# zhangyi-3/UCDIR

Measured on AMD Instinct MI355X. Metric: restored images/sec at 50-step p_sample_loop, 256x256 SID, higher is better.
Workload: dtype bf16

## Files before the change

### ucdir_amd/csrc/akgm_ws64.hip.h

```cpp
#pragma once
#include "asmops.hip.h"
#include "akgm_ws32.hip.h"

struct AkWs64 {
    static constexpr int NW = 8;
    static constexpr int HPOS = 272;
    static constexpr int HALO = HPOS * 128;
    static constexpr int HBYTES(int hpos) { return ((hpos + 15) / 16) * 2048; }
    static constexpr int PSTEP = 32 * 128;
    static constexpr int SEGB = 8 * NW;
    static constexpr int CPS = SEGB / 16;
    static constexpr int STAGE = 128 * SEGB;
    static constexpr int ATT = 128 * 32;
    static constexpr int TCS = 9 * 32 * NW * 4;
    static constexpr int NK = 36;
    static constexpr int lds(int hpos) { return 2 * HBYTES(hpos) + 2 * STAGE + 2 * ATT + TCS; }
};

template <int NPT, int NW, bool ASYM>
__global__ __launch_bounds__(64 * NW, 2) void akgm_ws64_kernel(const AkgmHP p) {
    static_assert(NW == AkWs64::NW && ASYM, "akgm_ws64_kernel: only the eight-wave kind with the chores on waves 0 - 3 is built");
    using L = AkWs64;
    constexpr int NK = L::NK;
    constexpr int CPX = 512;
    constexpr int NPX = 32 * NPT;
    constexpr int FEAT = 4 * NW;
    constexpr int PP = 1024 / L::SEGB;
    constexpr int NDW = 4;
    extern __shared__ __attribute__((aligned(16))) unsigned char smem[];
    const int tid = threadIdx.x, lane = tid & 63, l31 = lane & 31, hh = lane >> 5;
    const int wave = __builtin_amdgcn_readfirstlane(tid >> 6);
    int lid;
    {
        const int nblk = gridDim.x, bid = blockIdx.x;
        const int q = nblk >> 3, r = nblk & 7, xcd = bid & 7;
        lid = (xcd < r ? xcd * (q + 1) : r * (q + 1) + (xcd - r) * q) + (bid >> 3);
    }
#ifndef W64_DBGWAVE
#define W64_DBGWAVE (NW - 3)
#endif
#ifdef UCDIR_TIMING
    const bool dbg_on = p.dbg && (lid == (int)gridDim.x / 2 + 3) && (lane == 0) && (wave == W64_DBGWAVE);
    int dbg_n = 0;
#define W64_STAMP() do { if (dbg_on && dbg_n < 250) p.dbg[dbg_n++] = __builtin_amdgcn_s_memtime(); } while (0)
#else
#define W64_STAMP() do {} while (0)
#endif
    W64_STAMP();
    constexpr int NROLE = 512 / FEAT;
    const int nslots = (int)gridDim.x / NROLE;
    const int role = lid / nslots, slot = lid - role * nslots;
    const int Wp = p.Wp, Ptot = (p.H + 2) * Wp, Plast = p.H * Wp + p.W;
    const float inv_wp = 1.0f / (float)Wp;
    const int tps = p.tiles_x, T = p.nbatch * tps;
    const int t_beg = (int)((long long)slot * T / nslots), t_end = (int)((long long)(slot + 1) * T / nslots);
    if (t_beg >= t_end) return;
    const int chan0 = FEAT * role;
    const int gch0 = 64 * (chan0 >> 6);
    const int HB = p.tw;
    const unsigned OFF_STAGE = 2 * HB, OFF_ATT = OFF_STAGE + 2 * L::STAGE, OFF_TCS = OFF_ATT + 2 * L::ATT;

    bf16x8_t af[NK];
    {
        const unsigned char* Ab = reinterpret_cast<const unsigned char*>(p.A) + ((long long)(role * NW + wave) * NK) * 1024 + lane * 16;
#pragma unroll
        for (int j = 0; j < NK; ++j) af[j] = *reinterpret_cast<const bf16x8_t*>(Ab + j * 1024);
    }
#pragma unroll
    for (int j = 0; j < NK; ++j) asm volatile("" : "+v"(af[j]));
    W64_STAMP();

    const int npiece = (NPX + 2 * Wp + 2 + 7) >> 3;
    constexpr int NHOP = (L::HPOS / 8 + NDW - 1) / NDW;
    constexpr int NROP = NW / NDW;
    unsigned bt[9];
#pragma unroll
    for (int t = 0; t < 9; ++t) {
        const int hp = l31 + (t / 3) * Wp + t % 3;
        bt[t] = hp * 128 + ((hh ^ ((hp >> 1) & 7)) << 4) + HB;
    }
    const unsigned tc_lane = OFF_TCS + 4 * 8 * (4 * wave + 2 * hh);
    const unsigned att_lane = OFF_ATT + l31 * 32;
    const unsigned st_lane = OFF_STAGE + l31 * L::SEGB + (((wave >> 1) ^ ((l31 >> 2) & (L::CPS - 1))) << 4) + 8 * (wave & 1) + 4 * hh;

    int b = t_beg / tps, ti = t_beg - b * tps;
    auto dma_op = [&](auto opc, int nb, int nti, int buf) {
        constexpr int op = decltype(opc)::value;
        unsigned ln = lane;
        asm volatile("" : "+v"(ln));
        if constexpr (op < NHOP) {
            const int k = op * NDW + wave;
            if (k < npiece) {
                int sp = nti * NPX + 8 * k + (int)(ln >> 3);
                sp = sp < Ptot ? sp : Ptot - 1;
                const unsigned off = (unsigned)sp * (CPX * 2) + (unsigned)(gch0 + (((ln & 7) ^ (4 * (k & 1) + (ln >> 4))) << 3)) * 2;
                dma16_sbase(p.h + (long long)nb * p.h_bstride, off, (unsigned)__builtin_amdgcn_readfirstlane(buf * HB + k * 1024));
            }
        } else if constexpr (op == NHOP) {
            if (wave < NPT) {
                int P = Wp + 1 + nti * NPX + 32 * wave + (int)(ln >> 1); P = P < Ptot ? P : Ptot - 1;
                int y = fdiv_small(P, inv_wp), x = P - y * Wp;
                y = y < 1 ? 1 : (y > p.H ? p.H : y); x = x < 1 ? 1 : (x > p.W ? p.W : x);
                dma16_sbase(p.G + (long long)nb * p.g_bstride, (unsigned)((((y - 1) * p.W + (x - 1)) * 8 + (int)(ln & 1) * 4) * 4),
                          (unsigned)__builtin_amdgcn_readfirstlane(OFF_ATT + buf * L::ATT + wave * 1024));
            }
        } else {
            constexpr int rk = op - NHOP - 1;
            const int piece = NDW * rk + wave;
            if (piece < NPX / PP) {
                const unsigned pos = PP * piece + ln / L::CPS;
                int P = Wp + 1 + nti * NPX + (int)pos; P = P < Ptot ? P : Ptot - 1;
                const unsigned off = (unsigned)P * (CPX * 2) + (unsigned)(chan0 + (((ln & (L::CPS - 1)) ^ ((pos >> 2) & (L::CPS - 1))) << 3)) * 2;
                dma16_sbase(p.res + (long long)nb * p.res_bstride, off, (unsigned)__builtin_amdgcn_readfirstlane(OFF_STAGE + buf * L::STAGE + piece * 1024));
            }
        }
    };
    constexpr int NOPS = NHOP + 1 + NROP;
    if (wave < NDW) static_for<0, NOPS>([&](auto opc) { dma_op(opc, b, ti, 0); });

    int b_cur = -1;
    float rstd = 1.f, aw[8];
#pragma unroll
    for (int s = 0; s < 8; ++s) aw[s] = 0.f;
    stat_t S1 = 0, S2 = 0;
    bool have_prev = false;
    long long prev_out[NROP];
#pragma unroll
    for (int i = 0; i < NROP; ++i) prev_out[i] = -1;

#pragma unroll 1
    for (int t = t_beg; t <= t_end; ++t) {
        const int buf = (t - t_beg) & 1;
        W64_STAMP();
        asm volatile("s_waitcnt vmcnt(0) lgkmcnt(0)\n\ts_barrier" ::: "memory");
        W64_STAMP();
        if (have_prev && wave < NDW) {
#pragma unroll
            for (int i = 0; i < NROP; ++i) {
                if (prev_out[i] >= 0) {
                    const u32x4_t ln = *reinterpret_cast<const u32x4_t*>(smem + OFF_STAGE + (buf ^ 1) * L::STAGE + (i * 64 * NDW + tid) * 16);
                    *reinterpret_cast<u32x4_t*>(reinterpret_cast<unsigned char*>(p.out) + prev_out[i]) = ln;
                }
            }
        }
        if (t == t_end) break;
        if (b != b_cur) {
            if (b_cur >= 0 && p.stats_out) {
                const stat_t a = wave_sum_ll(S1), q2 = wave_sum_ll(S2);
                if (lane == 0) stat_add_fx(p.stats_out, b_cur, a, q2);
            }
            S1 = 0; S2 = 0;
            b_cur = b;
            float mean_b = 0.f;
            if (p.own_tc) stat_mean_rstd_wave(p.stats, b, p.inv_count, lane, mean_b, rstd);
            else rstd = __builtin_bit_cast(float, __builtin_amdgcn_readfirstlane(__builtin_bit_cast(int, p.ms[2 * b + 1])));
            const float inv_b = 1.0f / rstd;
#pragma unroll
            for (int i = 0; i < (9 + NW - 1) / NW; ++i) {
                const int pc = i * NW + wave;
                if (pc < 9) {
                    const long long rel = (long long)pc * (8 * CPX) + 8 * chan0 + lane * 4;
                    if (p.own_tc) akgm_tc_piece(p, rel, smem + OFF_TCS + pc * 1024 + lane * 16, inv_b, mean_b);
                    else __builtin_amdgcn_global_load_lds((const GLOBAL_AS void*)(p.Tc + (long long)b * 9 * (8 * CPX) + rel),
                                                          (LDS_AS void*)(smem + OFF_TCS + pc * 1024), 16, 0, 0);
                }
            }
#pragma unroll
            for (int s = 0; s < 8; ++s) aw[s] = __builtin_bit_cast(float, __builtin_amdgcn_readfirstlane(__builtin_bit_cast(int, p.attw[b * 8 + s])));
            asm volatile("s_waitcnt vmcnt(0) lgkmcnt(0)\n\ts_barrier" ::: "memory");
        }
        const bool last = t + 1 == t_end;
        int nb = b, nti = ti + 1;
        if (nti == tps) { nti = 0; ++nb; }
        asm volatile("s_waitcnt lgkmcnt(0)" ::: "memory");
        W64_STAMP();
        if (!last && wave < NDW) static_for<0, NOPS>([&](auto opc) { dma_op(opc, nb, nti, buf ^ 1); });

        const int P0 = Wp + 1 + ti * NPX;
        const unsigned ab0 = buf * L::ATT, sb0 = buf * L::STAGE;
#pragma unroll
        for (int k = 0; k < 9; ++k) bt[k] = buf ? bt[k] + HB : bt[k] - HB;
        float s1 = 0.f, s2 = 0.f;
#pragma unroll 1
        for (int qp = 0; qp < NPT; qp += 2) {
            f32x16_t acc[2];
            bool valid[2];
#pragma unroll
            for (int tq = 0; tq < 2; ++tq) {
                const int P = P0 + 32 * (qp + tq) + l31;
                const int y = fdiv_small(P, inv_wp), x = P - y * Wp;
                valid[tq] = x >= 1 && x <= p.W && P <= Plast;
                const int cy = (y <= 1) ? 0 : ((y >= p.H) ? 2 : 1);
                const int cx = (x <= 1) ? 0 : ((x >= p.W) ? 2 : 1);
                const unsigned tca = tc_lane + (cy * 3 + cx) * (128 * NW);
                acc[tq] = lds_read_f32x16(smem + tca);
            }
            bf16x8_t bfr[3][2];
            __builtin_amdgcn_sched_barrier(0);
            asm volatile("s_waitcnt lgkmcnt(0)" ::: "memory");
            W64_STAMP();
            auto frag = [&](auto jc, bf16x8_t (&dst)[2]) {
                constexpr int j = decltype(jc)::value;
                const unsigned a0 = bt[j >> 2] ^ ((j & 3) << 5);
                lds_read16_asm<0>(dst[0], a0);
                lds_read16_asm<L::PSTEP>(dst[1], a0);
            };
            frag(std::integral_constant<int, 0>{}, bfr[0]);
            frag(std::integral_constant<int, 1>{}, bfr[1]);
            __builtin_amdgcn_s_setprio(1);
            static_for<0, NK>([&](auto jc) {
                constexpr int j = decltype(jc)::value;
                if constexpr (j + 2 < NK) frag(std::integral_constant<int, j + 2>{}, bfr[(j + 2) % 3]);
                constexpr int younger = (j + 2 < NK) ? 4 : ((j + 1 < NK) ? 2 : 0);
                lgkm_wait_asm<younger>();
#pragma unroll
                for (int tq = 0; tq < 2; ++tq) acc[tq] = __builtin_amdgcn_mfma_f32_32x32x16_bf16(af[j], bfr[j % 3][tq], acc[tq], 0, 0, 0);
            });
            __builtin_amdgcn_s_setprio(0);
            W64_STAMP();
#pragma unroll
            for (int tq = 0; tq < 2; ++tq) {
                const unsigned aq = att_lane + ab0 + (qp + tq) * 1024;
                const f32x4_t a0 = *reinterpret_cast<const f32x4_t*>(smem + aq), a1 = *reinterpret_cast<const f32x4_t*>(smem + aq + 16);
                const float att[8] = {a0[0] * aw[0], a0[1] * aw[1], a0[2] * aw[2], a0[3] * aw[3], a1[0] * aw[4], a1[1] * aw[5], a1[2] * aw[6], a1[3] * aw[7]};
                float o2[2];
#pragma unroll
                for (int k = 0; k < 2; ++k) {
                    float sa = 0.f;
#pragma unroll
                    for (int s = 0; s < 8; ++s) sa += att[s] * acc[tq][8 * k + s];
                    o2[k] = rstd * sa;
                }
                const unsigned sa = st_lane + sb0 + (qp + tq) * (32 * L::SEGB);
                const unsigned rv = *reinterpret_cast<const unsigned*>(smem + sa);
                float v0 = silu_fast(o2[0]) + __builtin_bit_cast(float, rv << 16);
                float v1 = silu_fast(o2[1]) + __builtin_bit_cast(float, rv & 0xffff0000u);
                *reinterpret_cast<unsigned*>(smem + sa) = pack2_bf16(v0, v1);
                v0 = valid[tq] ? v0 : 0.f; v1 = valid[tq] ? v1 : 0.f;
                s1 += v0 + v1; s2 += v0 * v0 + v1 * v1;
            }
#pragma unroll
            for (int k = 0; k < 9; ++k) bt[k] += 2 * L::PSTEP;
        }
#pragma unroll
        for (int k = 0; k < 9; ++k) bt[k] -= NPT * L::PSTEP;
        S1 += stat_fx((double)s1); S2 += stat_fx((double)s2);
        have_prev = true;
        if (wave < NDW) {
#pragma unroll
            for (int i = 0; i < NROP; ++i) {
                const int it = i * 64 * NDW + tid, mpos = it / L::CPS, P = P0 + mpos;
                const int y = fdiv_small(P < Ptot ? P : Ptot - 1, inv_wp), x = P - y * Wp;
                const bool ok = mpos < NPX && x >= 1 && x <= p.W && P <= Plast;
                prev_out[i] = ok ? ((long long)b * p.out_bstride + (long long)P * CPX + chan0 + (((it & (L::CPS - 1)) ^ ((mpos >> 2) & (L::CPS - 1))) << 3)) * 2 : -1;
            }
        }
        b = nb; ti = nti;
    }
#ifdef UCDIR_TIMING
    if (dbg_on) p.dbg[255] = dbg_n;
#endif
    if (p.stats_out) {
        const stat_t a = wave_sum_ll(S1), q2 = wave_sum_ll(S2);
        if (lane == 0) stat_add_fx(p.stats_out, b_cur, a, q2);
    }
}
```

### ucdir_amd/csrc/pack.h

```cpp
#pragma once
#include <cmath>
#include <cstdint>
#include <vector>

#include "common.h"

struct PackedConv {
    std::vector<bf16_t> A;
    std::vector<float> bias;
    std::vector<float> Tb, Tg;
    int rows_pad = 0, Kpad = 0, ntaps = 0, cin = 0, cout = 0, ncls = 0;
};

static inline bool tap_valid(int cls, int tap) {
    const int cy = cls / 3, cx = cls % 3, ky = tap / 3, kx = tap % 3;
    if (cy == 0 && ky == 0) return false;
    if (cy == 2 && ky == 2) return false;
    if (cx == 0 && kx == 0) return false;
    if (cx == 2 && kx == 2) return false;
    return true;
}

static inline PackedConv pack_conv(const float* w, const float* bias, const float* gamma, const float* beta,
                                   int cout, int cin, int ks, int TM) {
    PackedConv P;
    P.ntaps = ks * ks; P.cin = cin; P.cout = cout;
    P.Kpad = ((P.ntaps * cin + 63) / 64) * 64;
    P.rows_pad = ((cout + TM - 1) / TM) * TM;
    P.A.assign((size_t)P.rows_pad * P.Kpad, 0);
    P.bias.assign(P.rows_pad, 0.f);
    if (bias) for (int o = 0; o < cout; ++o) P.bias[o] = bias[o];
    P.ncls = (ks == 3) ? 9 : 1;
    const bool fold = gamma != nullptr;
    std::vector<double> wb((size_t)P.ntaps * cout, 0.0), wg((size_t)P.ntaps * cout, 0.0);
    for (int o = 0; o < cout; ++o)
        for (int c = 0; c < cin; ++c)
            for (int t = 0; t < P.ntaps; ++t) {
                const float wv = w[((size_t)o * cin + c) * P.ntaps + t];
                const float ws = fold ? wv * gamma[c] : wv;
                const bf16_t q = f2bf(ws);
                P.A[(size_t)o * P.Kpad + (size_t)t * cin + c] = q;
                if (fold) {
                    wb[(size_t)t * cout + o] += (double)wv * beta[c];
                    wg[(size_t)t * cout + o] += (double)bf2f(q);
                }
            }
    if (fold) {
        P.Tb.assign((size_t)P.ncls * cout, 0.f);
        P.Tg.assign((size_t)P.ncls * cout, 0.f);
        for (int cls = 0; cls < P.ncls; ++cls)
            for (int o = 0; o < cout; ++o) {
                double sb = 0, sg = 0;
                for (int t = 0; t < P.ntaps; ++t) {
                    const int t9 = (P.ntaps == 9) ? t : 4;
                    if (P.ncls == 9 && !tap_valid(cls, t9)) continue;
                    sb += wb[(size_t)t * cout + o]; sg += wg[(size_t)t * cout + o];
                }
                P.Tb[(size_t)cls * cout + o] = (float)sb;
                P.Tg[(size_t)cls * cout + o] = (float)sg;
            }
    }
    return P;
}

static inline std::vector<bf16_t> pack_conv_ws(const PackedConv& P) {
    std::vector<bf16_t> img((size_t)2 * 36 * 2 * 32 * 8, 0);
    for (int rw = 0; rw < 2; ++rw)
        for (int j = 0; j < 36; ++j)
            for (int hk = 0; hk < 2; ++hk)
                for (int rho = 0; rho < 32; ++rho) {
                    const int o = 32 * rw + 16 * ((rho >> 2) & 1) + (rho & 3) + 4 * (rho >> 3);
                    const int tap = j >> 2, c0 = 16 * (j & 3) + 8 * hk;
                    for (int e = 0; e < 8; ++e)
                        img[((((size_t)rw * 36 + j) * 2 + hk) * 32 + rho) * 8 + e] = P.A[(size_t)o * P.Kpad + (size_t)tap * 64 + c0 + e];
                }
    return img;
}

static inline std::vector<bf16_t> pack_conv_ws128(const std::vector<bf16_t>& A10) {
    const int K10 = 10 * 128, nj = 80;
    std::vector<bf16_t> img((size_t)2 * nj * 2 * 32 * 8, 0);
    for (int rw = 0; rw < 2; ++rw)
        for (int j = 0; j < nj; ++j)
            for (int hk = 0; hk < 2; ++hk)
                for (int rho = 0; rho < 32; ++rho) {
                    const int o = 32 * rw + 16 * ((rho >> 2) & 1) + (rho & 3) + 4 * (rho >> 3);
                    const int tap = j >> 3, c0 = 16 * (j & 7) + 8 * hk;
                    const size_t dst = j < 72 ? ((((size_t)rw * 72 + j) * 2 + hk) * 32 + rho) * 8
                                              : (size_t)2 * 72 * 2 * 32 * 8 + ((((size_t)rw * 8 + (j - 72)) * 2 + hk) * 32 + rho) * 8;
                    for (int e = 0; e < 8; ++e) img[dst + e] = A10[(size_t)o * K10 + (size_t)tap * 128 + c0 + e];
                }
    return img;
}

static inline std::vector<bf16_t> pack_conv_res10(const PackedConv& P, const float* wres) {
    const int cin = P.cin, K10 = 10 * cin;
    std::vector<bf16_t> A((size_t)P.rows_pad * K10, 0);
    for (int o = 0; o < P.rows_pad; ++o) {
        for (int k = 0; k < 9 * cin; ++k) A[(size_t)o * K10 + k] = P.A[(size_t)o * P.Kpad + k];
        if (o < P.cout)
            for (int c = 0; c < cin; ++c) A[(size_t)o * K10 + 9 * cin + c] = f2bf(wres[(size_t)o * cin + c]);
    }
    return A;
}

struct PackedAkgm {
    std::vector<bf16_t> A;
    std::vector<float> bias;
    std::vector<float> Tb, Tg;
    int C = 0, cg = 0, Kpad = 0;
};

static inline PackedAkgm pack_akgm(const float* wsp, const float* bsp, const float* gamma, const float* beta, int C,
                                   int kpad_override = 0) {
    PackedAkgm P;
    P.C = C; P.cg = C / 8;
    const int cg = P.cg;
    const bool chunked = (cg == 64) && !kpad_override;
    P.Kpad = kpad_override ? kpad_override : (chunked ? 640 : ((9 * cg + 63) / 64) * 64);
    P.A.assign((size_t)8 * C * P.Kpad, 0);
    P.bias.assign((size_t)8 * C, 0.f);
    P.Tb.assign((size_t)9 * 8 * C, 0.f);
    P.Tg.assign((size_t)9 * 8 * C, 0.f);
    for (int o = 0; o < 8 * C; ++o) P.bias[o] = bsp[o];
    for (int g = 0; g < 8; ++g)
        for (int pr = 0; pr < C; ++pr) {
            const int t32 = pr / 32, rho = pr % 32;
            const int floc = 4 * t32 + ((rho >> 4) & 1) * 2 + ((rho >> 2) & 1);
            const int s = (rho & 3) + 4 * ((rho >> 3) & 1);
            const int o = g * C + 8 * floc + s;
            bf16_t* row = &P.A[((size_t)g * C + pr) * P.Kpad];
            double wb[9] = {0}, wg[9] = {0};
            for (int ci = 0; ci < cg; ++ci) {
                const int cglob = g * cg + ci;
                for (int t = 0; t < 9; ++t) {
                    const float wv = wsp[((size_t)o * cg + ci) * 9 + t];
                    const bf16_t q = f2bf(wv * gamma[cglob]);
                    row[chunked ? (size_t)(ci / 32) * 320 + (size_t)t * 32 + (ci % 32) : (size_t)t * cg + ci] = q;
                    wb[t] += (double)wv * beta[cglob];
                    wg[t] += (double)bf2f(q);
                }
            }
            for (int cls = 0; cls < 9; ++cls) {
                double sb = 0, sg = 0;
                for (int t = 0; t < 9; ++t) if (tap_valid(cls, t)) { sb += wb[t]; sg += wg[t]; }
                P.Tb[(size_t)cls * 8 * C + o] = (float)sb;
                P.Tg[(size_t)cls * 8 * C + o] = (float)sg;
            }
        }
    return P;
}

static inline std::vector<bf16_t> pack_akgm_pre(const float* wsp, const float* gamma, int C) {
    const int cg = C / 8;
    const int nk16 = (cg == 8) ? 5 : 9;
    const int nunits = C / 16;
    std::vector<bf16_t> img((size_t)nunits * nk16 * 2 * 128 * 8, 0);
    for (int U = 0; U < nunits; ++U)
        for (int R = 0; R < 128; ++R) {
            const int t32 = R >> 5, rho = R & 31;
            const int hr = (rho >> 2) & 1, q = (rho >> 4) & 1, s = (rho & 3) + 4 * ((rho >> 3) & 1);
            const int c = U * 16 + 4 * t32 + 2 * hr + q;
            const int g = c / cg;
            const int o = 8 * c + s;
            for (int j = 0; j < nk16; ++j)
                for (int hk = 0; hk < 2; ++hk)
                    for (int e = 0; e < 8; ++e) {
                        const int tap = (cg == 8) ? 2 * j + hk : j;
                        const int ci = (cg == 8) ? e : 8 * hk + e;
                        if (tap > 8) continue;
                        img[(((size_t)U * nk16 + j) * 2 + hk) * 1024 + (size_t)R * 8 + e] =
                            f2bf(wsp[((size_t)o * cg + ci) * 9 + tap] * gamma[g * cg + ci]);
                    }
        }
    return img;
}

static inline std::vector<bf16_t> pack_qkv_ws(const PackedConv& P, int C) {
    const int RT = 3 * C / 256, NKS = C / 16;
    std::vector<bf16_t> img((size_t)RT * 8 * NKS * 2 * 32 * 8, 0);
    for (int rt = 0; rt < RT; ++rt)
        for (int w = 0; w < 8; ++w)
            for (int rho = 0; rho < 32; ++rho) {
                const bool v = rt * 256 >= 2 * C;
                const int R = 256 * rt + 32 * w + (v ? rho : 16 * ((rho >> 2) & 1) + 4 * (rho >> 3) + (rho & 3));
                for (int j = 0; j < NKS; ++j)
                    for (int hh = 0; hh < 2; ++hh)
                        for (int e = 0; e < 8; ++e)
                            img[(((((size_t)rt * 8 + w) * NKS + j) * 2 + hh) * 32 + rho) * 8 + e] = P.A[(size_t)R * P.Kpad + 16 * j + 8 * hh + e];
            }
    return img;
}

static inline std::vector<bf16_t> pack_conv_tiled(const PackedConv& P, int TM) {
    const int TPS = 256 / TM, nsteps = (9 + TPS - 1) / TPS, nch = P.cin / 32, nrt = P.rows_pad / TM, ipt = TM / 16;
    std::vector<bf16_t> img((size_t)nrt * nch * nsteps * 8192, 0);
    for (int rt = 0; rt < nrt; ++rt)
        for (int c = 0; c < nch; ++c)
            for (int u = 0; u < nsteps; ++u)
                for (int k = 0; k < 16; ++k)
                    for (int lane = 0; lane < 64; ++lane) {
                        const int row = (k % ipt) * 16 + (lane >> 2);
                        int tap = TPS * u + k / ipt; tap = tap < 9 ? tap : 8;
                        const int lc = (lane & 3) ^ ((row >> 2) & 3);
                        const bf16_t* src = &P.A[(size_t)(rt * TM + row) * P.Kpad + (size_t)tap * P.cin + c * 32 + lc * 8];
                        bf16_t* dst = &img[((((size_t)rt * nch + c) * nsteps + u) * 16 + k) * 512 + lane * 8];
                        for (int e = 0; e < 8; ++e) dst[e] = src[e];
                    }
    return img;
}

static inline std::vector<bf16_t> pack_conv_sk(const std::vector<bf16_t>& A, int npar, int rows_pad, int Kld, int cin, int ntaps, int MW) {
    const int ROWS = 128 * MW, nrt = (rows_pad + ROWS - 1) / ROWS, nch = cin / 32, nf = 4 * MW;
    std::vector<bf16_t> img((size_t)npar * nrt * nch * ntaps * nf * 2 * 512 + (size_t)4 * nf * 2 * 512, 0);
    for (int par = 0; par < npar; ++par)
        for (int rt = 0; rt < nrt; ++rt)
            for (int c = 0; c < nch; ++c)
                for (int t = 0; t < ntaps; ++t)
                    for (int f = 0; f < nf; ++f)
                        for (int j = 0; j < 2; ++j)
                            for (int lane = 0; lane < 64; ++lane) {
                                const int rho = lane & 31, hh = lane >> 5;
                                const int row = rt * ROWS + 32 * f + 16 * ((rho >> 2) & 1) + (rho & 3) + 4 * (rho >> 3);
                                if (row >= rows_pad) continue;
                                const bf16_t* src = &A[((size_t)par * rows_pad + row) * Kld + (size_t)t * cin + 32 * c + 16 * j + 8 * hh];
                                bf16_t* dst = &img[(((((((size_t)par * nrt + rt) * nch + c) * ntaps + t) * nf + f) * 2 + j) * 64 + lane) * 8];
                                for (int e = 0; e < 8; ++e) dst[e] = src[e];
                            }
    return img;
}

static inline std::vector<bf16_t> pack_akgm_ws32(const float* wsp, const float* gamma, int C) {
    const int cg = C / 8, nk = 18, nb = C / 32;
    std::vector<bf16_t> img((size_t)nb * 8 * nk * 2 * 32 * 8, 0);
    for (int blk = 0; blk < nb; ++blk)
        for (int w = 0; w < 8; ++w)
            for (int rho = 0; rho < 32; ++rho) {
                const int c4 = 2 * ((rho >> 2) & 1) + (rho >> 4), sm = 4 * ((rho >> 3) & 1) + (rho & 3);
                const int c = 32 * blk + 4 * w + c4, o = 8 * c + sm, g = c / cg;
                for (int j = 0; j < nk; ++j)
                    for (int hk = 0; hk < 2; ++hk)
                        for (int e = 0; e < 8; ++e) {
                            const int tap = j >> 1, ci = 16 * (j & 1) + 8 * hk + e;
                            img[(((((size_t)blk * 8 + w) * nk + j) * 2 + hk) * 32 + rho) * 8 + e] = f2bf(wsp[((size_t)o * cg + ci) * 9 + tap] * gamma[g * cg + ci]);
                        }
            }
    return img;
}

static inline std::vector<bf16_t> pack_akgm_ws64(const float* wsp, const float* gamma, int C) {
    const int cg = C / 8, nk = 36, nh = C / 32;
    std::vector<bf16_t> img((size_t)nh * 8 * nk * 2 * 32 * 8, 0);
    for (int hg = 0; hg < nh; ++hg)
        for (int w = 0; w < 8; ++w)
            for (int rho = 0; rho < 32; ++rho) {
                const int c4 = 2 * ((rho >> 2) & 1) + (rho >> 4), sm = 4 * ((rho >> 3) & 1) + (rho & 3);
                const int c = 32 * hg + 4 * w + c4, o = 8 * c + sm, g = c / cg;
                for (int j = 0; j < nk; ++j)
                    for (int hk = 0; hk < 2; ++hk)
                        for (int e = 0; e < 8; ++e) {
                            const int tap = j >> 2, ci = 16 * (j & 3) + 8 * hk + e;
                            img[(((((size_t)hg * 8 + w) * nk + j) * 2 + hk) * 32 + rho) * 8 + e] = f2bf(wsp[((size_t)o * cg + ci) * 9 + tap] * gamma[g * cg + ci]);
                        }
            }
    return img;
}

static inline std::vector<bf16_t> pack_stem_frags(const std::vector<float>& t, const std::vector<float>& bias, int cin, int C0) {
    const int nb = C0 / 64;
    std::vector<bf16_t> f((size_t)nb * 2 * 5 * 64 * 8, 0);
    for (int cb = 0; cb < nb; ++cb)
        for (int tm = 0; tm < 2; ++tm)
            for (int j = 0; j < 5; ++j)
                for (int lane = 0; lane < 64; ++lane) {
                    const int row = cb * 64 + tm * 32 + (lane & 31), tap = 2 * j + (lane >> 5);
                    bf16_t* d = &f[((((size_t)cb * 2 + tm) * 5 + j) * 64 + lane) * 8];
                    if (tap > 8) {
                        const bf16_t hi = f2bf(bias[row]);
                        d[0] = hi; d[1] = f2bf(bias[row] - bf2f(hi));
                        continue;
                    }
                    for (int e = 0; e < cin; ++e) d[e] = f2bf(t[(size_t)(tap * cin + e) * C0 + row]);
                }
    return f;
}

static inline std::vector<bf16_t> pack_final_frags(const float* w, int cout, int C) {
    const int nc = C / 32;
    std::vector<bf16_t> f((size_t)9 * nc * 64 * 8, 0);
    for (int tap = 0; tap < 9; ++tap)
        for (int c32 = 0; c32 < nc; ++c32)
            for (int lane = 0; lane < 64; ++lane) {
                const int row = lane & 15, g = lane >> 4;
                if (row >= cout) continue;
                for (int e = 0; e < 8; ++e)
                    f[(((size_t)tap * nc + c32) * 64 + lane) * 8 + e] = f2bf(w[((size_t)row * C + c32 * 32 + g * 8 + e) * 9 + tap]);
            }
    return f;
}

static inline PackedConv pack_upconv(const float* w, const float* bias, int cout, int cin, int TM) {
    PackedConv P;
    P.ntaps = 4; P.cin = cin; P.cout = cout; P.ncls = 1;
    P.Kpad = 4 * cin;
    P.rows_pad = ((cout + TM - 1) / TM) * TM;
    P.A.assign((size_t)4 * P.rows_pad * P.Kpad, 0);
    P.bias.assign(P.rows_pad, 0.f);
    if (bias) for (int o = 0; o < cout; ++o) P.bias[o] = bias[o];
    auto in_set = [](int par, int d, int k) { return par == 0 ? (d == 0 ? k == 0 : k >= 1) : (d == 0 ? k <= 1 : k == 2); };
    for (int py = 0; py < 2; ++py) for (int px = 0; px < 2; ++px)
        for (int o = 0; o < cout; ++o) for (int c = 0; c < cin; ++c)
            for (int dy = 0; dy < 2; ++dy) for (int dx = 0; dx < 2; ++dx) {
                double sum = 0;
                for (int ky = 0; ky < 3; ++ky) for (int kx = 0; kx < 3; ++kx)
                    if (in_set(py, dy, ky) && in_set(px, dx, kx)) sum += w[((size_t)o * cin + c) * 9 + ky * 3 + kx];
                P.A[((size_t)(py * 2 + px) * P.rows_pad + o) * P.Kpad + (size_t)(dy * 2 + dx) * cin + c] = f2bf((float)sum);
            }
    return P;
}
```

Measured before the change: 37.28.

## Switch ws64 adaptive conv from 32x32x16 to 16x16x32 bf16 MFMA tiles

Restructures the ws64 kernel's inner GEMM to use 16x16x32 MFMA instructions instead of 32x32x16. This changes the lane mapping, the LDS swizzle, the halo DMA channel ordering, the epilogue and the host weight packing to fit the new tile shape. B fragments now flow through a 5-deep ring, each lane ends up with one output channel instead of two, and residual stores become 16-bit. The aim is better MFMA throughput or scheduling, paid for with more instructions and more LDS reads per tile, narrower epilogue stores, and a risk of bank conflicts from the new swizzle.

```diff
diff --git a/ucdir_amd/csrc/akgm_ws64.hip.h b/ucdir_amd/csrc/akgm_ws64.hip.h
--- a/ucdir_amd/csrc/akgm_ws64.hip.h
+++ b/ucdir_amd/csrc/akgm_ws64.hip.h
@@ -8,12 +8,14 @@
     static constexpr int HALO = HPOS * 128;
     static constexpr int HBYTES(int hpos) { return ((hpos + 15) / 16) * 2048; }
     static constexpr int PSTEP = 32 * 128;
+    static constexpr int PT16 = 16 * 128;
     static constexpr int SEGB = 8 * NW;
     static constexpr int CPS = SEGB / 16;
     static constexpr int STAGE = 128 * SEGB;
     static constexpr int ATT = 128 * 32;
     static constexpr int TCS = 9 * 32 * NW * 4;
-    static constexpr int NK = 36;
+    static constexpr int NK32 = 18;
+    static constexpr int NK = 2 * NK32;
     static constexpr int lds(int hpos) { return 2 * HBYTES(hpos) + 2 * STAGE + 2 * ATT + TCS; }
 };
 
@@ -28,7 +30,7 @@
     constexpr int PP = 1024 / L::SEGB;
     constexpr int NDW = 4;
     extern __shared__ __attribute__((aligned(16))) unsigned char smem[];
-    const int tid = threadIdx.x, lane = tid & 63, l31 = lane & 31, hh = lane >> 5;
+    const int tid = threadIdx.x, lane = tid & 63, col = lane & 15, kb = lane >> 4;
     const int wave = __builtin_amdgcn_readfirstlane(tid >> 6);
     int lid;
     {
@@ -76,12 +78,12 @@
     unsigned bt[9];
 #pragma unroll
     for (int t = 0; t < 9; ++t) {
-        const int hp = l31 + (t / 3) * Wp + t % 3;
-        bt[t] = hp * 128 + ((hh ^ ((hp >> 1) & 7)) << 4) + HB;
-    }
-    const unsigned tc_lane = OFF_TCS + 4 * 8 * (4 * wave + 2 * hh);
-    const unsigned att_lane = OFF_ATT + l31 * 32;
-    const unsigned st_lane = OFF_STAGE + l31 * L::SEGB + (((wave >> 1) ^ ((l31 >> 2) & (L::CPS - 1))) << 4) + 8 * (wave & 1) + 4 * hh;
+        const int hp = col + (t / 3) * Wp + t % 3;
+        bt[t] = hp * 128 + ((kb ^ (((hp >> 1) & 3) << 1)) << 4) + HB;
+    }
+    const unsigned tc_lane = OFF_TCS + 4 * 8 * (4 * wave + kb);
+    const unsigned att_lane = OFF_ATT + col * 32;
+    const unsigned st_lane = OFF_STAGE + col * L::SEGB + (((wave >> 1) ^ ((col >> 2) & (L::CPS - 1))) << 4) + 8 * (wave & 1) + 2 * kb;
 
     int b = t_beg / tps, ti = t_beg - b * tps;
     auto dma_op = [&](auto opc, int nb, int nti, int buf) {
@@ -93,7 +95,7 @@
             if (k < npiece) {
                 int sp = nti * NPX + 8 * k + (int)(ln >> 3);
                 sp = sp < Ptot ? sp : Ptot - 1;
-                const unsigned off = (unsigned)sp * (CPX * 2) + (unsigned)(gch0 + (((ln & 7) ^ (4 * (k & 1) + (ln >> 4))) << 3)) * 2;
+                const unsigned off = (unsigned)sp * (CPX * 2) + (unsigned)(gch0 + (((ln & 7) ^ ((ln >> 4) << 1)) << 3)) * 2;
                 dma16_sbase(p.h + (long long)nb * p.h_bstride, off, (unsigned)__builtin_amdgcn_readfirstlane(buf * HB + k * 1024));
             }
         } else if constexpr (op == NHOP) {
@@ -183,61 +185,54 @@
         float s1 = 0.f, s2 = 0.f;
 #pragma unroll 1
         for (int qp = 0; qp < NPT; qp += 2) {
-            f32x16_t acc[2];
-            bool valid[2];
-#pragma unroll
-            for (int tq = 0; tq < 2; ++tq) {
-                const int P = P0 + 32 * (qp + tq) + l31;
+            f32x4_t acc[2][4];
+            bool valid[4];
+#pragma unroll
+            for (int q = 0; q < 4; ++q) {
+                const int P = P0 + 32 * qp + 16 * q + col;
                 const int y = fdiv_small(P, inv_wp), x = P - y * Wp;
-                valid[tq] = x >= 1 && x <= p.W && P <= Plast;
+                valid[q] = x >= 1 && x <= p.W && P <= Plast;
                 const int cy = (y <= 1) ? 0 : ((y >= p.H) ? 2 : 1);
                 const int cx = (x <= 1) ? 0 : ((x >= p.W) ? 2 : 1);
                 const unsigned tca = tc_lane + (cy * 3 + cx) * (128 * NW);
-                acc[tq] = lds_read_f32x16(smem + tca);
-            }
-            bf16x8_t bfr[3][2];
+                acc[0][q] = *reinterpret_cast<const f32x4_t*>(smem + tca);
+                acc[1][q] = *reinterpret_cast<const f32x4_t*>(smem + tca + 16);
+            }
+            constexpr int NB = 4 * L::NK32, RING = 5;
+            bf16x8_t bfr[RING];
             __builtin_amdgcn_sched_barrier(0);
             asm volatile("s_waitcnt lgkmcnt(0)" ::: "memory");
             W64_STAMP();
-            auto frag = [&](auto jc, bf16x8_t (&dst)[2]) {
-                constexpr int j = decltype(jc)::value;
-                const unsigned a0 = bt[j >> 2] ^ ((j & 3) << 5);
-                lds_read16_asm<0>(dst[0], a0);
-                lds_read16_asm<L::PSTEP>(dst[1], a0);
+            auto frag = [&](auto nc) {
+                constexpr int n = decltype(nc)::value, j = n >> 2;
+                lds_read16_asm<(n & 3) * L::PT16>(bfr[n % RING], bt[j >> 1] ^ ((j & 1) << 6));
             };
-            frag(std::integral_constant<int, 0>{}, bfr[0]);
-            frag(std::integral_constant<int, 1>{}, bfr[1]);
+            static_for<0, RING - 1>([&](auto nc) { frag(nc); });
             __builtin_amdgcn_s_setprio(1);
-            static_for<0, NK>([&](auto jc) {
-                constexpr int j = decltype(jc)::value;
-                if constexpr (j + 2 < NK) frag(std::integral_constant<int, j + 2>{}, bfr[(j + 2) % 3]);
-                constexpr int younger = (j + 2 < NK) ? 4 : ((j + 1 < NK) ? 2 : 0);
+            static_for<0, NB>([&](auto nc) {
+                constexpr int n = decltype(nc)::value, j = n >> 2, q = n & 3;
+                if constexpr (n + RING - 1 < NB) frag(std::integral_constant<int, n + RING - 1>{});
+                constexpr int younger = (n + RING - 1 < NB) ? RING - 1 : NB - 1 - n;
                 lgkm_wait_asm<younger>();
 #pragma unroll
-                for (int tq = 0; tq < 2; ++tq) acc[tq] = __builtin_amdgcn_mfma_f32_32x32x16_bf16(af[j], bfr[j % 3][tq], acc[tq], 0, 0, 0);
+                for (int rt = 0; rt < 2; ++rt) acc[rt][q] = __builtin_amdgcn_mfma_f32_16x16x32_bf16(af[2 * j + rt], bfr[n % RING], acc[rt][q], 0, 0, 0);
             });
             __builtin_amdgcn_s_setprio(0);
             W64_STAMP();
 #pragma unroll
-            for (int tq = 0; tq < 2; ++tq) {
-                const unsigned aq = att_lane + ab0 + (qp + tq) * 1024;
+            for (int q = 0; q < 4; ++q) {
+                const unsigned aq = att_lane + ab0 + (2 * qp + q) * 512;
                 const f32x4_t a0 = *reinterpret_cast<const f32x4_t*>(smem + aq), a1 = *reinterpret_cast<const f32x4_t*>(smem + aq + 16);
                 const float att[8] = {a0[0] * aw[0], a0[1] * aw[1], a0[2] * aw[2], a0[3] * aw[3], a1[0] * aw[4], a1[1] * aw[5], a1[2] * aw[6], a1[3] * aw[7]};
-                float o2[2];
-#pragma unroll
-                for (int k = 0; k < 2; ++k) {
-                    float sa = 0.f;
-#pragma unroll
-                    for (int s = 0; s < 8; ++s) sa += att[s] * acc[tq][8 * k + s];
-                    o2[k] = rstd * sa;
-                }
-                const unsigned sa = st_lane + sb0 + (qp + tq) * (32 * L::SEGB);
-                const unsigned rv = *reinterpret_cast<const unsigned*>(smem + sa);
-                float v0 = silu_fast(o2[0]) + __builtin_bit_cast(float, rv << 16);
-                float v1 = silu_fast(o2[1]) + __builtin_bit_cast(float, rv & 0xffff0000u);
-                *reinterpret_cast<unsigned*>(smem + sa) = pack2_bf16(v0, v1);
-                v0 = valid[tq] ? v0 : 0.f; v1 = valid[tq] ? v1 : 0.f;
-                s1 += v0 + v1; s2 += v0 * v0 + v1 * v1;
+                float sa = 0.f;
+#pragma unroll
+                for (int s = 0; s < 8; ++s) sa += att[s] * acc[s >> 2][q][s & 3];
+                const unsigned sta = st_lane + sb0 + (2 * qp + q) * (16 * L::SEGB);
+                const unsigned rv = *reinterpret_cast<const unsigned short*>(smem + sta);
+                float v = silu_fast(rstd * sa) + __builtin_bit_cast(float, rv << 16);
+                *reinterpret_cast<unsigned short*>(smem + sta) = (unsigned short)pack2_bf16(v, 0.f);
+                v = valid[q] ? v : 0.f;
+                s1 += v; s2 += v * v;
             }
 #pragma unroll
             for (int k = 0; k < 9; ++k) bt[k] += 2 * L::PSTEP;
diff --git a/ucdir_amd/csrc/pack.h b/ucdir_amd/csrc/pack.h
--- a/ucdir_amd/csrc/pack.h
+++ b/ucdir_amd/csrc/pack.h
@@ -249,20 +249,20 @@
 }
 
 static inline std::vector<bf16_t> pack_akgm_ws64(const float* wsp, const float* gamma, int C) {
-    const int cg = C / 8, nk = 36, nh = C / 32;
-    std::vector<bf16_t> img((size_t)nh * 8 * nk * 2 * 32 * 8, 0);
+    const int cg = C / 8, nk = 18, nh = C / 32;
+    std::vector<bf16_t> img((size_t)nh * 8 * nk * 2 * 4 * 16 * 8, 0);
     for (int hg = 0; hg < nh; ++hg)
         for (int w = 0; w < 8; ++w)
-            for (int rho = 0; rho < 32; ++rho) {
-                const int c4 = 2 * ((rho >> 2) & 1) + (rho >> 4), sm = 4 * ((rho >> 3) & 1) + (rho & 3);
-                const int c = 32 * hg + 4 * w + c4, o = 8 * c + sm, g = c / cg;
-                for (int j = 0; j < nk; ++j)
-                    for (int hk = 0; hk < 2; ++hk)
-                        for (int e = 0; e < 8; ++e) {
-                            const int tap = j >> 2, ci = 16 * (j & 3) + 8 * hk + e;
-                            img[(((((size_t)hg * 8 + w) * nk + j) * 2 + hk) * 32 + rho) * 8 + e] = f2bf(wsp[((size_t)o * cg + ci) * 9 + tap] * gamma[g * cg + ci]);
-                        }
-            }
+            for (int rt = 0; rt < 2; ++rt)
+                for (int r = 0; r < 16; ++r) {
+                    const int c = 32 * hg + 4 * w + (r >> 2), o = 8 * c + 4 * rt + (r & 3), g = c / cg;
+                    for (int j = 0; j < nk; ++j)
+                        for (int kb = 0; kb < 4; ++kb)
+                            for (int e = 0; e < 8; ++e) {
+                                const int tap = j >> 1, ci = 32 * (j & 1) + 8 * kb + e;
+                                img[((((((size_t)hg * 8 + w) * nk + j) * 2 + rt) * 4 + kb) * 16 + r) * 8 + e] = f2bf(wsp[((size_t)o * cg + ci) * 9 + tap] * gamma[g * cg + ci]);
+                            }
+                }
     return img;
 }
 
```

Result: no change. 36.98 (-0.8%).
